# ChanghyeonKim93/nonlinear_optimizer_for_slam

Measured on AMD Instinct MI355X. Metric: ndt6_gauss_newton_residual_blocks_per_sec, higher is better.
Workload: dtype f64

## Files before the change

nonlinear_optimizer_for_slam_amd/csrc/assemble_one_launch.hpp:

```cpp
#pragma once

#include "assemble_pass.hpp"

namespace nos {

constexpr size_t kSingleBlockMaxElements = size_t(1024) * 15;

template <typename Problem, typename T, int BLOCK, bool NT>
__device__ __forceinline__ int single_block_loop(const TiledLayout& L, typename Problem::Params& P, uint32_t n_chunks,
                                                 LmDevice& s_lm, double* s_sum, double* __restrict__ cost_history,
                                                 int history_capacity) {
  constexpr int kF = Problem::kFields;
  constexpr int kOut = Problem::kOut;
  const T* __restrict__ base = static_cast<const T*>(L.base);
  int executed = 0;
  while (s_lm.st.done == 0) {
    set_pose(P, &s_lm);
    T acc[kOut];
#pragma unroll
    for (int k = 0; k < kOut; ++k) acc[k] = T(0);
    constexpr uint32_t kRound = (kF * sizeof(T) > 64) ? 2 : 4;
    for (uint32_t c = 0; c < n_chunks; c += kRound) {
      T x[kRound][kF][1];
      uint64_t i0[kRound];
#pragma unroll
      for (uint32_t u = 0; u < kRound; ++u) {
        const uint32_t cu = (c + u < n_chunks) ? c + u : c;
        i0[u] = uint64_t(cu) * BLOCK + threadIdx.x;
        const uint64_t off = (i0[u] >> L.tile_shift) * L.tile_stride + (i0[u] & L.tile_mask);
#pragma unroll
        for (int f = 0; f < kF; ++f) load_items<T, 1, NT>(base + field_offset<Problem>(L, i0[u], off, f), x[u][f]);
      }
      __builtin_amdgcn_sched_barrier(0);
#pragma unroll
      for (uint32_t u = 0; u < kRound; ++u) {
        if (c + u < n_chunks) {
          T xi[kF];
#pragma unroll
          for (int f = 0; f < kF; ++f) xi[f] = x[u][f][0];
          Problem::item(xi, P, i0[u] < L.n, acc);
        }
      }
    }
    double dacc[kOut];
#pragma unroll
    for (int k = 0; k < kOut; ++k) dacc[k] = double(acc[k]);
    block_reduce_store<kOut, BLOCK>(dacc, s_sum, false);
    __syncthreads();
    if (threadIdx.x == 0) {
      if (cost_history != nullptr && executed < history_capacity)
        __hip_atomic_store(cost_history + executed, s_sum[kOut - 1], __ATOMIC_RELAXED, __HIP_MEMORY_SCOPE_SYSTEM);
      lm_step_lane<kOut>(lds_ptr(s_sum), lds_ptr(&s_lm));
    }
    ++executed;
    __syncthreads();
  }
  return executed;
}

template <typename Problem, typename T, int BLOCK, bool NT = false>
__global__ __launch_bounds__(BLOCK) void solve_single_block_kernel(TiledLayout L, typename Problem::Params P,
                                                                  uint32_t n_chunks, LmDevice* lm,
                                                                  double* __restrict__ cost_history, int history_capacity,
                                                                  double* entry_host, unsigned long long* seq_host,
                                                                  unsigned long long seq) {
  constexpr int kOut = Problem::kOut;
  __shared__ double s_lm_raw[(sizeof(LmDevice) + 7) / 8];
  LmDevice& s_lm = *reinterpret_cast<LmDevice*>(s_lm_raw);
  __shared__ double s_sum[kLmTotDoubles(kOut)];
  if (threadIdx.x == 0) s_lm = *lm;
  __syncthreads();
  const int executed = single_block_loop<Problem, T, BLOCK, NT>(L, P, n_chunks, s_lm, s_sum, cost_history, history_capacity);
  if (threadIdx.x < kOut && entry_host != nullptr && executed > 0)
    __hip_atomic_store(entry_host + kLogOut + threadIdx.x, s_sum[threadIdx.x], __ATOMIC_RELAXED, __HIP_MEMORY_SCOPE_SYSTEM);
  if (threadIdx.x == 0) {
    const nos_host::LmState st = s_lm.st;
    lm->st = st;
    if (entry_host != nullptr) {
#pragma unroll
      for (int k = 0; k < 9; ++k)
        __hip_atomic_store(entry_host + kLogR + k, st.R[k], __ATOMIC_RELAXED, __HIP_MEMORY_SCOPE_SYSTEM);
#pragma unroll
      for (int k = 0; k < 3; ++k)
        __hip_atomic_store(entry_host + kLogT + k, st.t[k], __ATOMIC_RELAXED, __HIP_MEMORY_SCOPE_SYSTEM);
      __hip_atomic_store(entry_host + kLogLambda, st.lambda, __ATOMIC_RELAXED, __HIP_MEMORY_SCOPE_SYSTEM);
      __hip_atomic_store(entry_host + kLogPrevCost, st.previous_cost, __ATOMIC_RELAXED, __HIP_MEMORY_SCOPE_SYSTEM);
      __hip_atomic_store(entry_host + kLogCost, st.cost, __ATOMIC_RELAXED, __HIP_MEMORY_SCOPE_SYSTEM);
      __hip_atomic_store(entry_host + kLogIteration, double(st.iteration), __ATOMIC_RELAXED, __HIP_MEMORY_SCOPE_SYSTEM);
      __hip_atomic_store(entry_host + kLogDone, double(st.done), __ATOMIC_RELAXED, __HIP_MEMORY_SCOPE_SYSTEM);
      __hip_atomic_store(entry_host + kLogOk, double(st.ok), __ATOMIC_RELAXED, __HIP_MEMORY_SCOPE_SYSTEM);
      __hip_atomic_store(entry_host + kLogExecuted, double(executed), __ATOMIC_RELAXED, __HIP_MEMORY_SCOPE_SYSTEM);
    }
  }
  if (threadIdx.x < kWave) {
    asm volatile("s_waitcnt vmcnt(0)" ::: "memory");
    if (threadIdx.x == 0 && seq_host != nullptr) {
      __builtin_amdgcn_fence(__ATOMIC_RELEASE, "");
      asm volatile("s_waitcnt vmcnt(0)" ::: "memory");
      __hip_atomic_store(seq_host, seq, __ATOMIC_RELAXED, __HIP_MEMORY_SCOPE_SYSTEM);
    }
  }
}

constexpr uint32_t kClusterMaxBlocks = 256;
constexpr unsigned long long kClusterTimeoutTicks = 5000000ull;
constexpr unsigned long long kClusterMailboxTimeoutTicks = kMailboxTimeoutTicks;

struct ClusterCtl {
  unsigned int abort;
  unsigned int pad0[31];
  struct alignas(128) Arrival {
    unsigned int count;
    unsigned int pad[31];
  } arrival[8];
};

__device__ __forceinline__ double sc1_load(const double* p) {
  return __hip_atomic_load(p, __ATOMIC_RELAXED, __HIP_MEMORY_SCOPE_AGENT);
}
__device__ __forceinline__ void sc1_store(double* p, double v) {
  __hip_atomic_store(p, v, __ATOMIC_RELAXED, __HIP_MEMORY_SCOPE_AGENT);
}

__device__ __forceinline__ void state_store_sc1(LmDevice* lm, const nos_host::LmState& st) {
  double* d = reinterpret_cast<double*>(&lm->st);
  const double* s = reinterpret_cast<const double*>(&st);
  constexpr int kWords = int(sizeof(nos_host::LmState) / sizeof(double));
  static_assert(sizeof(nos_host::LmState) % sizeof(double) == 0, "LmState must be a whole number of doubles");
#pragma unroll
  for (int k = 0; k < kWords; ++k) sc1_store(d + k, s[k]);
}
__device__ __forceinline__ void state_load_sc1(const LmDevice* lm, nos_host::LmState& st) {
  const double* d = reinterpret_cast<const double*>(&lm->st);
  double* s = reinterpret_cast<double*>(&st);
  constexpr int kWords = int(sizeof(nos_host::LmState) / sizeof(double));
#pragma unroll
  for (int k = 0; k < kWords; ++k) s[k] = sc1_load(d + k);
}

template <int FIELDS, int ELEM>
struct ResidentShape;
template <>
struct ResidentShape<15, 8> { static constexpr int RI = 3, LI = 3; };
template <>
struct ResidentShape<15, 4> { static constexpr int RI = 3, LI = 4; };
template <>
struct ResidentShape<5, 8> { static constexpr int RI = 9, LI = 7; };
template <>
struct ResidentShape<5, 4> { static constexpr int RI = 10, LI = 14; };

template <typename Problem, typename T>
struct StreamRegRounds { static constexpr int kRR = 3; };
template <int LOSS>
struct StreamRegRounds<Ndt6Problem<float, LOSS>, float> { static constexpr int kRR = 0; };
constexpr int kStreamRegRoundsMax = 3;

template <typename Problem, typename T, int BLOCK, int RI, int LI, int SI = 0, bool SPF = false, bool NT = false>
__global__ __launch_bounds__(BLOCK) void solve_cluster_kernel(TiledLayout L, typename Problem::Params P,
                                                             double* __restrict__ partials, LmDevice* lm, ClusterCtl* ctl,
                                                             double* __restrict__ cost_history, int history_capacity,
                                                             double* entry_host, unsigned long long* seq_host,
                                                             unsigned long long seq, uint32_t items_per_lane,
                                                             const Mailbox* mail = nullptr, uint32_t stream_lds = 0u,
                                                             uint32_t stream_reg = 0u) {
  constexpr int kF = Problem::kFields;
  constexpr int kOut = Problem::kOut;
  constexpr int kCols = 32;
  constexpr int kSlices = BLOCK / kCols;
  const T* __restrict__ base = static_cast<const T*>(L.base);
  constexpr int kRF = kF;
  extern __shared__ __align__(16) unsigned char resident_raw[];
  T* resident = reinterpret_cast<T*>(resident_raw);
  __shared__ int s_flag;
  __shared__ int s_fast;
  __shared__ double red[kSlices][kCols];
  __shared__ double s_tot[kLmTotDoubles(kOut)];
  __shared__ double s_lmd_raw[(sizeof(LmDevice) + 7) / 8];
  LmDevice& s_lmd = *reinterpret_cast<LmDevice*>(s_lmd_raw);
  nos_host::LmState& s_state = s_lmd.st;
  [[maybe_unused]] __shared__ double s_local[kCols];
  [[maybe_unused]] __shared__ unsigned long long s_round0;
  const bool multi = mail != nullptr;

  const uint32_t J = items_per_lane & 0x7fffffffu;
  [[maybe_unused]] const bool allow_fast = (items_per_lane >> 31) == 0u;
  [[maybe_unused]] constexpr int kXccCol = 28;
  [[maybe_unused]] const unsigned int my_xcc = xcc_id();
  const uint64_t block_base = uint64_t(blockIdx.x) * BLOCK * J;
  auto fetch = [&](uint32_t j, T (&dst)[kRF]) -> bool {
    const uint64_t i = block_base + uint64_t(j) * BLOCK + threadIdx.x;
    const bool ok = i < L.n;
    const uint64_t ic = ok ? i : 0;
    const uint64_t off = (ic >> L.tile_shift) * L.tile_stride + (ic & L.tile_mask);
    T xt[kF][1];
#pragma unroll
    for (int f = 0; f < kF; ++f) load_items<T, 1, false>(base + field_offset<Problem>(L, ic, off, f), xt[f]);
#pragma unroll
    for (int f = 0; f < kF; ++f) dst[f] = ok ? xt[f][0] : T(0);
    return ok;
  };
  auto evaluate_resident = [&](const T (&xi)[kRF], bool ok, T (&acc_)[kOut]) { Problem::item(xi, P, ok, acc_); };
  T x[RI > 0 ? RI : 1][kRF];
  bool valid[RI > 0 ? RI : 1];
  static_assert(SI == 0 || (RI == 0 && LI == 0), "the streaming form keeps nothing resident");
  constexpr int kSI = SI > 0 ? SI : 1;
  [[maybe_unused]] T xs[kF][kSI];
  [[maybe_unused]] uint64_t xs_i0 = 0;
  [[maybe_unused]] constexpr int kRR = (SI > 0 && !SPF) ? StreamRegRounds<Problem, T>::kRR : 0;
  static_assert(kRR <= kStreamRegRoundsMax, "the option's range covers every instantiation");
  [[maybe_unused]] T xr[kRR > 0 ? kRR : 1][kF][kSI];
  [[maybe_unused]] const uint32_t my_rounds = blockIdx.x < J ? (J - blockIdx.x + gridDim.x - 1) / gridDim.x : 0u;
  [[maybe_unused]] const uint32_t lds_k = SI > 0 ? min(stream_lds, my_rounds > 0u ? my_rounds - 1u : 0u) : 0u;
  [[maybe_unused]] const uint32_t reg_k = kRR > 0 ? min(min(stream_reg, uint32_t(kRR)), (my_rounds > 0u ? my_rounds - 1u : 0u) - lds_k) : 0u;
  [[maybe_unused]] const uint32_t alt_k = min(lds_k, reg_k);
  [[maybe_unused]] auto chip_round = [&](uint32_t i) -> uint32_t {
    return uint32_t(uint64_t(i + 1u) * my_rounds / (lds_k + reg_k + 1u));
  };
  [[maybe_unused]] auto lds_slot_round = [&](uint32_t sl) -> uint32_t {
    return sl < lds_k ? chip_round(sl < alt_k ? 2u * sl : alt_k + sl) : ~0u;
  };
  [[maybe_unused]] const uint32_t lds_r0 = lds_slot_round(0u);
  [[maybe_unused]] const uint32_t lds_r1 = lds_slot_round(1u);
  [[maybe_unused]] const uint32_t lds_r2 = lds_slot_round(2u);
  [[maybe_unused]] uint32_t reg_r[kRR > 0 ? kRR : 1];
#pragma unroll
  for (int j = 0; j < (kRR > 0 ? kRR : 1); ++j)
    reg_r[j] = uint32_t(j) < reg_k ? chip_round(uint32_t(j) < alt_k ? 2u * uint32_t(j) + 1u : alt_k + uint32_t(j)) : ~0u;
#pragma unroll
  for (int j = 0; j < (kRR > 0 ? kRR : 1); ++j)
#pragma unroll
    for (int f = 0; f < kF; ++f)
#pragma unroll
      for (int e = 0; e < kSI; ++e) xr[j][f][e] = T(0);
  [[maybe_unused]] auto lds_round = [&](uint32_t s) -> uint32_t { return s == 0u ? lds_r0 : s == 1u ? lds_r1 : s == 2u ? lds_r2 : ~0u; };
  [[maybe_unused]] auto fetch_chunk = [&](uint32_t c, T (&dst)[kF][kSI]) -> uint64_t {
    const uint64_t i0 = uint64_t(c) * (uint64_t(BLOCK) * kSI) + uint64_t(threadIdx.x) * kSI;
    const uint64_t off = (i0 >> L.tile_shift) * L.tile_stride + (i0 & L.tile_mask);
#pragma unroll
    for (int f = 0; f < kF; ++f) load_items<T, kSI, NT>(base + field_offset<Problem>(L, i0, off, f), dst[f]);
    return i0;
  };
  if constexpr (SI > 0) {
    if (blockIdx.x < J) xs_i0 = fetch_chunk(blockIdx.x, xs);
  }
#pragma unroll
  for (int j = 0; j < RI; ++j) {
    valid[j] = false;
    if (uint32_t(j) < J) {
      valid[j] = fetch(uint32_t(j), x[j]);
    } else {
#pragma unroll
      for (int f = 0; f < kRF; ++f) x[j][f] = T(0);
    }
  }
  if constexpr (LI > 0) {
    for (uint32_t j = RI; j < J; ++j) {
      T xi[kRF];
      (void)fetch(j, xi);
#pragma unroll
      for (int f = 0; f < kRF; ++f) resident[(size_t(j - RI) * kRF + f) * BLOCK + threadIdx.x] = xi[f];
    }
  }
  NOS_PROBE(if (threadIdx.x < 4) s_step_cycles[threadIdx.x] = 0ull;)
  if (threadIdx.x == 0) {
    s_lmd.settings = lm->settings;
    s_state = lm->st;
    s_flag = s_state.done != 0 ? 1 : 0;
    s_fast = 0;
    if (__hip_atomic_load(&ctl->abort, __ATOMIC_RELAXED, __HIP_MEMORY_SCOPE_AGENT) != 0u) s_flag = 2;
    if (multi && blockIdx.x == 0) s_round0 = *mail->round;
  }
  __syncthreads();
  [[maybe_unused]] const unsigned int group = blockIdx.x & 7u;
  const unsigned int n_groups = gridDim.x < 8u ? gridDim.x : 8u;
  unsigned int it = 0;
  int executed = 0;
  NOS_PROBE(unsigned long long tq[6] = {0, 0, 0, 0, 0, 0}, tp = 0;)
#define NOS_RES_STAMP(slot_) NOS_PROBE({ const unsigned long long now_ = wall_clock64(); tq[slot_] += now_ - tp; tp = now_; })
  while (s_flag == 0) {
    NOS_PROBE(tp = wall_clock64();)
    if constexpr (kOut == 28) {
#pragma unroll
      for (int k = 0; k < 9; ++k) P.R[k] = T(uniform_load(&s_state.R[k]));
#pragma unroll
      for (int k = 0; k < 3; ++k) P.t[k] = T(uniform_load(&s_state.t[k]));
    } else {
#pragma unroll
      for (int k = 0; k < 4; ++k) P.R2[k] = T(uniform_load(&s_state.R[k]));
#pragma unroll
      for (int k = 0; k < 2; ++k) P.t2[k] = T(uniform_load(&s_state.t[k]));
    }
    T acc[kOut];
#pragma unroll
    for (int k = 0; k < kOut; ++k) acc[k] = T(0);
    if constexpr (SI > 0) {
      const uint32_t n_chunks = J;
      auto evaluate = [&](const T (&xc)[kF][SI > 0 ? SI : 1], uint64_t i0) {
#pragma unroll
        for (int it = 0; it < (SI > 0 ? SI : 1); ++it) {
          T xi[kF];
#pragma unroll
          for (int f = 0; f < kF; ++f) xi[f] = xc[f][it];
          Problem::item(xi, P, (i0 + it) < L.n, acc);
        }
      };
      if constexpr (SPF) {
        for (uint32_t c = blockIdx.x; c < n_chunks; c += gridDim.x) {
          T xb[kF][SI > 0 ? SI : 1];
          uint64_t i1 = 0;
          const uint32_t cn = c + gridDim.x;
          if (cn < n_chunks) i1 = fetch_chunk(cn, xb);
          evaluate(xs, xs_i0);
#pragma unroll
          for (int f = 0; f < kF; ++f)
#pragma unroll
            for (int it = 0; it < (SI > 0 ? SI : 1); ++it) xs[f][it] = xb[f][it];
          xs_i0 = i1;
        }
      } else {
        auto lds_at = [&](uint32_t s, int f, int e) -> T& {
          return resident[((size_t(s) * kF + f) * BLOCK + threadIdx.x) * kSI + e];
        };
        auto evaluate_lds = [&](uint32_t s, uint32_t cl) {
          const uint64_t i0 = uint64_t(cl) * (uint64_t(BLOCK) * kSI) + uint64_t(threadIdx.x) * kSI;
#pragma unroll
          for (int e = 0; e < kSI; ++e) {
            T xi[kF];
#pragma unroll
            for (int f = 0; f < kF; ++f) xi[f] = lds_at(s, f, e);
            Problem::item(xi, P, (i0 + e) < L.n, acc);
          }
        };
        const bool on_chip = it != 0u;
        uint32_t s = 0;
        uint32_t next_res = lds_round(0u);
        auto in_registers = [&](uint32_t r) -> bool {
          bool hit = false;
#pragma unroll
          for (int j = 0; j < kRR; ++j) hit = hit || r == reg_r[j];
          return hit;
        };
        uint32_t k = 0;
        if constexpr (kRR == 0) {
          while (k < my_rounds) {
            __builtin_amdgcn_sched_barrier(0);
            if (!on_chip && k == next_res) {
#pragma unroll
              for (int f = 0; f < kF; ++f)
#pragma unroll
                for (int e = 0; e < kSI; ++e) lds_at(s, f, e) = xs[f][e];
              next_res = lds_round(++s);
            }
            evaluate(xs, xs_i0);
            uint32_t kn = k + 1u;
            if (on_chip)
              for (uint32_t sn = s; kn == lds_round(sn); ++sn) ++kn;
            xs_i0 = fetch_chunk(blockIdx.x + (kn < my_rounds ? kn : 0u) * gridDim.x, xs);
            for (uint32_t kr = k + 1u; kr < kn; ++kr) {
              evaluate_lds(s, blockIdx.x + kr * gridDim.x);
              next_res = lds_round(++s);
            }
            k = kn;
          }
        } else
#pragma unroll
        for (int j = 0; j <= kRR; ++j) {
          const uint32_t rj = j < kRR ? reg_r[j < kRR ? j : 0] : ~0u;
          const uint32_t stop = min(rj, my_rounds);
          const uint32_t hi = (!on_chip && rj != ~0u) ? rj + 1u : stop;
          auto lds_rounds_below = [&](uint32_t lim) {
            while (next_res < lim) {
              evaluate_lds(s, blockIdx.x + next_res * gridDim.x);
              next_res = lds_round(++s);
            }
          };
          if (on_chip && j > 0) lds_rounds_below(min(k, stop));
          while (k < hi) {
            __builtin_amdgcn_sched_barrier(0);
            if (!on_chip) {
              if (k == next_res) {
#pragma unroll
                for (int f = 0; f < kF; ++f)
#pragma unroll
                  for (int e = 0; e < kSI; ++e) lds_at(s, f, e) = xs[f][e];
                next_res = lds_round(++s);
              }
              if constexpr (kRR > 0) {
                if (j < kRR && k == rj) {
#pragma unroll
                  for (int f = 0; f < kF; ++f)
#pragma unroll
                    for (int e = 0; e < kSI; ++e) xr[j < kRR ? j : 0][f][e] = xs[f][e];
                }
              }
            }
            evaluate(xs, xs_i0);
            uint32_t kn = k + 1u;
            if (on_chip) {
              for (uint32_t sn = s;;) {
                if (kn == lds_round(sn)) {
                  ++sn;
                  ++kn;
                } else if (in_registers(kn)) {
                  ++kn;
                } else {
                  break;
                }
              }
            }
            xs_i0 = fetch_chunk(blockIdx.x + (kn < my_rounds ? kn : 0u) * gridDim.x, xs);
            if (on_chip) lds_rounds_below(min(kn, stop));
            k = kn;
          }
          if constexpr (kRR > 0) {
            if (j < kRR && on_chip && rj != ~0u)
              evaluate(xr[j < kRR ? j : 0], uint64_t(blockIdx.x + rj * gridDim.x) * (uint64_t(BLOCK) * kSI) + uint64_t(threadIdx.x) * kSI);
          }
        }
      }
      if constexpr (SPF) {
        if (blockIdx.x < n_chunks) xs_i0 = fetch_chunk(blockIdx.x, xs);
      }
    } else
    if (sizeof(T) == 8 && J >= uint32_t(RI)) {
#pragma unroll
      for (int j = 0; j < RI; ++j) evaluate_resident(x[j], valid[j], acc);
    } else {
#pragma unroll
      for (int j = 0; j < RI; ++j)
        if (uint32_t(j) < J) evaluate_resident(x[j], valid[j], acc);
    }
    if constexpr (LI > 0) {
      for (uint32_t j = RI; j < J; ++j) {
        T xi[kRF];
#pragma unroll
        for (int f = 0; f < kRF; ++f) xi[f] = resident[(size_t(j - RI) * kRF + f) * BLOCK + threadIdx.x];
        evaluate_resident(xi, (block_base + uint64_t(j) * BLOCK + threadIdx.x) < L.n, acc);
      }
    }
    double dacc[kOut];
#pragma unroll
    for (int k = 0; k < kOut; ++k) dacc[k] = double(acc[k]);
    NOS_RES_STAMP(0)
    {
      TaggedUnit* const block_units = reinterpret_cast<TaggedUnit*>(partials);
      TaggedUnit* const group_units = block_units + size_t(kClusterMaxBlocks) * 32;
      const unsigned long long tag = (seq << 24) | ((unsigned long long)it + 1ull);
      const double mine = block_reduce_value<kOut, BLOCK>(dacc);
      const bool probe = it == 0u && allow_fast;
      if (threadIdx.x < kOut) {
        if (s_fast != 0)
          tagged_store_plain(block_units + size_t(blockIdx.x) * 32 + threadIdx.x, mine, tag);
        else
          tagged_store(block_units + size_t(blockIdx.x) * 32 + threadIdx.x, mine, tag);
      } else if (probe && threadIdx.x == kXccCol) {
        tagged_store(block_units + size_t(blockIdx.x) * 32 + kXccCol, double(my_xcc), tag);
      }
      NOS_RES_STAMP(1)
      const unsigned long long deadline = wall_clock64() + (multi ? kClusterMailboxTimeoutTicks : kClusterTimeoutTicks);
      auto await = [&](const TaggedUnit* u, double* value) -> bool {
        unsigned int polls = 0;
        for (;;) {
          const TaggedUnit got = tagged_load(u);
          if (got.seq == tag) {
            *value = got.value;
            return true;
          }
          if ((++polls & 63u) == 0u &&
              (__hip_atomic_load(&ctl->abort, __ATOMIC_RELAXED, __HIP_MEMORY_SCOPE_AGENT) != 0u || wall_clock64() > deadline)) {
            __hip_atomic_store(&ctl->abort, 1u, __ATOMIC_RELAXED, __HIP_MEMORY_SCOPE_AGENT);
            s_flag = 2;
            return false;
          }
        }
      };
      const int col = threadIdx.x % kCols;
      const int slice = threadIdx.x / kCols;
      if (blockIdx.x < n_groups) {
        const unsigned int g_size = (gridDim.x - blockIdx.x + 7u) >> 3;
        double gsum = 0.0;
        for (unsigned int m0 = 0; m0 < g_size; m0 += kSlices) {
          const unsigned int m = m0 + slice;
          double v = 0.0;
          if (m < g_size && (col < kOut || (probe && col == kXccCol))) {
            (void)await(block_units + size_t(blockIdx.x + 8u * m) * 32 + col, &v);
            if (col == kXccCol) v = v == double(my_xcc) ? 0.0 : 1.0;
          }
          red[slice][col] = v;
          __syncthreads();
          if (threadIdx.x < kOut || (probe && threadIdx.x == kXccCol)) {
#pragma unroll
            for (int sl = 0; sl < kSlices; ++sl) gsum += red[sl][threadIdx.x];
          }
          __syncthreads();
        }
        if ((threadIdx.x < kOut || (probe && threadIdx.x == kXccCol)) && s_flag != 2)
          tagged_store(group_units + (size_t(it & 1u) * 8 + blockIdx.x) * 32 + threadIdx.x, gsum, tag);
      }
      if (!multi || blockIdx.x == 0) {
        double v = 0.0;
        if (slice < int(n_groups) && (col < kOut || (probe && col == kXccCol)) && s_flag != 2)
          (void)await(group_units + (size_t(it & 1u) * 8 + slice) * 32 + col, &v);
        if (slice < 8) red[slice][col] = v;
      }
      __syncthreads();
      if (multi) {
        TaggedUnit* const global_units = group_units + size_t(2) * 8 * 32;
        if (blockIdx.x == 0) {
          if (threadIdx.x < kCols && s_flag != 2) {
            double tot = 0.0;
            if (threadIdx.x < kOut || (probe && threadIdx.x == kXccCol))
              for (unsigned int g = 0; g < n_groups; ++g) tot += red[g][threadIdx.x];
            s_local[threadIdx.x] = tot;
          }
          __syncthreads();
          if (threadIdx.x < kWave) {
            const Mailbox mb = *mail;
            const unsigned long long round = s_round0 + (unsigned long long)it + 1ull;
            const unsigned int xtag = (unsigned int)(round % 0xFFFFFFFFull) + 1u;
            const size_t parity = size_t(round & 1ull);
            const size_t units_base = size_t(mb.n_ranks) * 2 * kMailSlotDoubles;
            const int lane = int(threadIdx.x);
            const bool giving_up = s_flag == 2;
            unsigned long long* const own = reinterpret_cast<unsigned long long*>(mb.peers[mb.rank] + units_base);
            if (giving_up) {
              if (lane < mb.n_ranks)
                __hip_atomic_store(reinterpret_cast<unsigned long long*>(mb.peers[lane] + units_base) +
                                       (size_t(mb.rank) * 2 + parity) * kMailSlotDoubles + 63,
                                   (unsigned long long)xtag << 32, __ATOMIC_RELAXED, __HIP_MEMORY_SCOPE_SYSTEM);
            } else {
              unsigned long long gran = 0ull;
              if (lane < 2 * kOut) {
                const unsigned long long bits = (unsigned long long)__double_as_longlong(s_local[lane >> 1]);
                gran = ((unsigned long long)xtag << 32) | ((lane & 1) ? (bits >> 32) : (bits & 0xFFFFFFFFull));
                for (int p = 0; p < mb.n_ranks; ++p)
                  __hip_atomic_store(reinterpret_cast<unsigned long long*>(mb.peers[p] + units_base) +
                                         (size_t(mb.rank) * 2 + parity) * kMailSlotDoubles + lane,
                                     gran, __ATOMIC_RELAXED, __HIP_MEMORY_SCOPE_SYSTEM);
              }
              double sum = 0.0;
              bool lost = false;
              const unsigned long long give_up_at = wall_clock64() + kClusterMailboxTimeoutTicks;
              for (int r = 0; r < mb.n_ranks && !lost; ++r) {
                const unsigned long long* slot_r = own + (size_t(r) * 2 + parity) * kMailSlotDoubles;
                unsigned long long got = 0ull;
                unsigned int polls = 0;
                for (;;) {
                  if (lane < 2 * kOut) got = __hip_atomic_load(slot_r + lane, __ATOMIC_RELAXED, __HIP_MEMORY_SCOPE_SYSTEM);
                  const bool here = lane >= 2 * kOut || (unsigned int)(got >> 32) == xtag;
                  if (__ballot(!here) == 0ull) break;
                  if ((++polls & 15u) == 0u) {
                    const unsigned long long peer_gave_up =
                        __hip_atomic_load(slot_r + 63, __ATOMIC_RELAXED, __HIP_MEMORY_SCOPE_SYSTEM);
                    if ((unsigned int)(peer_gave_up >> 32) == xtag || wall_clock64() > give_up_at ||
                        __hip_atomic_load(&ctl->abort, __ATOMIC_RELAXED, __HIP_MEMORY_SCOPE_AGENT) != 0u) {
                      lost = true;
                      break;
                    }
                  }
                  __builtin_amdgcn_s_sleep(1);
                }
                const unsigned int half = (unsigned int)(got & 0xFFFFFFFFull);
                const unsigned int other = (unsigned int)__shfl_xor(int(half), 1, kWave);
                const double value = __longlong_as_double((long long)(((unsigned long long)((lane & 1) ? half : other) << 32) |
                                                                      (unsigned long long)((lane & 1) ? other : half)));
                sum += value;
              }
              if (lost) {
                if (lane == 0) {
                  __hip_atomic_store(&ctl->abort, 1u, __ATOMIC_RELAXED, __HIP_MEMORY_SCOPE_AGENT);
                  s_flag = 2;
                }
                if (lane < mb.n_ranks)
                  __hip_atomic_store(reinterpret_cast<unsigned long long*>(mb.peers[lane] + units_base) +
                                         (size_t(mb.rank) * 2 + parity) * kMailSlotDoubles + 63,
                                     (unsigned long long)xtag << 32, __ATOMIC_RELAXED, __HIP_MEMORY_SCOPE_SYSTEM);
              } else if (lane < 2 * kOut && (lane & 1) == 0) {
                s_local[lane >> 1] = sum;
              }
            }
          }
          __syncthreads();
          if (s_flag != 2) {
            if (threadIdx.x < kOut || (probe && threadIdx.x == kXccCol))
              tagged_store(global_units + size_t(it & 1u) * 32 + threadIdx.x, s_local[threadIdx.x], tag);
          }
        }
        {
          double v = 0.0;
          if (threadIdx.x < kCols && (col < kOut || (probe && col == kXccCol)) && s_flag != 2)
            (void)await(global_units + size_t(it & 1u) * 32 + col, &v);
          if (threadIdx.x < kCols) red[0][col] = v;
        }
        __syncthreads();
      }
      NOS_RES_STAMP(2)
      if (s_flag == 2) break;
      if (multi) {
        if (threadIdx.x < kOut)
          s_tot[threadIdx.x] = red[0][threadIdx.x];
        else if (probe && threadIdx.x == kXccCol)
          s_fast = red[0][kXccCol] == 0.0 ? 1 : 0;
      } else
      if (threadIdx.x < kOut) {
        double tot = 0.0;
        for (unsigned int g = 0; g < n_groups; ++g) tot += red[g][threadIdx.x];
        s_tot[threadIdx.x] = tot;
      } else if (probe && threadIdx.x == kXccCol) {
        double strangers = 0.0;
        for (unsigned int g = 0; g < n_groups; ++g) strangers += red[g][kXccCol];
        s_fast = strangers == 0.0 ? 1 : 0;
      }
      __syncthreads();
    }
    {
      NOS_RES_STAMP(3)
      if (threadIdx.x == 0) {
        if (blockIdx.x == 0 && cost_history != nullptr && executed < history_capacity)
          __hip_atomic_store(cost_history + executed, s_tot[kOut - 1], __ATOMIC_RELAXED, __HIP_MEMORY_SCOPE_SYSTEM);
        lm_step_lane<kOut>(lds_ptr(s_tot), lds_ptr(&s_lmd));
        s_flag = s_state.done != 0 ? 1 : 0;
      }
    }
    ++executed;
    ++it;
    __syncthreads();
    NOS_RES_STAMP(4)
  }
  NOS_PROBE(
  if (blockIdx.x == 0 && threadIdx.x == 0 && entry_host != nullptr) {
    for (int k = 0; k < 5; ++k)
      __hip_atomic_store(entry_host + 50 + k, double(tq[k]) / double(executed > 0 ? executed : 1), __ATOMIC_RELAXED,
                         __HIP_MEMORY_SCOPE_SYSTEM);
    for (int k = 0; k < 3; ++k)
      __hip_atomic_store(entry_host + 56 + k, double(s_step_cycles[k]) / double(executed > 0 ? executed : 1), __ATOMIC_RELAXED,
                         __HIP_MEMORY_SCOPE_SYSTEM);
  }
  )
  if (s_flag == 1 && blockIdx.x == 0) {
    if (threadIdx.x < kOut && entry_host != nullptr && executed > 0)
      __hip_atomic_store(entry_host + kLogOut + threadIdx.x, s_tot[threadIdx.x], __ATOMIC_RELAXED, __HIP_MEMORY_SCOPE_SYSTEM);
    if (threadIdx.x == 0) {
      const nos_host::LmState st = s_state;
      lm->st = st;
      if (multi) *mail->round = s_round0 + (unsigned long long)executed;
      if (entry_host != nullptr) {
#pragma unroll
        for (int k = 0; k < 9; ++k)
          __hip_atomic_store(entry_host + kLogR + k, st.R[k], __ATOMIC_RELAXED, __HIP_MEMORY_SCOPE_SYSTEM);
#pragma unroll
        for (int k = 0; k < 3; ++k)
          __hip_atomic_store(entry_host + kLogT + k, st.t[k], __ATOMIC_RELAXED, __HIP_MEMORY_SCOPE_SYSTEM);
        __hip_atomic_store(entry_host + kLogLambda, st.lambda, __ATOMIC_RELAXED, __HIP_MEMORY_SCOPE_SYSTEM);
        __hip_atomic_store(entry_host + kLogPrevCost, st.previous_cost, __ATOMIC_RELAXED, __HIP_MEMORY_SCOPE_SYSTEM);
        __hip_atomic_store(entry_host + kLogCost, st.cost, __ATOMIC_RELAXED, __HIP_MEMORY_SCOPE_SYSTEM);
        __hip_atomic_store(entry_host + kLogIteration, double(st.iteration), __ATOMIC_RELAXED, __HIP_MEMORY_SCOPE_SYSTEM);
        __hip_atomic_store(entry_host + kLogDone, double(st.done), __ATOMIC_RELAXED, __HIP_MEMORY_SCOPE_SYSTEM);
        __hip_atomic_store(entry_host + kLogOk, double(st.ok), __ATOMIC_RELAXED, __HIP_MEMORY_SCOPE_SYSTEM);
        __hip_atomic_store(entry_host + kLogExecuted, double(executed), __ATOMIC_RELAXED, __HIP_MEMORY_SCOPE_SYSTEM);
      }
    }
    if (threadIdx.x < kWave) {
      asm volatile("s_waitcnt vmcnt(0)" ::: "memory");
      if (threadIdx.x == 0 && seq_host != nullptr) {
        __builtin_amdgcn_fence(__ATOMIC_RELEASE, "");
        asm volatile("s_waitcnt vmcnt(0)" ::: "memory");
        __hip_atomic_store(seq_host, seq, __ATOMIC_RELAXED, __HIP_MEMORY_SCOPE_SYSTEM);
      }
    }
  }
}

}
```

Before: 76.60 billion.

## Use single merged streaming loop for register/LDS-resident rounds in NDT kernels

Adds a single-loop path for NDT3 and NDT6 problems. On the first iteration it stashes chunks into LDS or register slots. On later iterations it walks all rounds in order, interleaving reads from LDS and registers with prefetched global chunks, instead of running a separate loop segment per register round. It also turns on one register-resident round for float NDT6. The aim is to cut loop-segment overhead and keep the global prefetch overlapped, at the cost of more register pressure and dynamic selection among the register slots.

Result: no change. 76.93 billion (median of 4 runs) (+0.4%).

```diff
diff --git a/nonlinear_optimizer_for_slam_amd/csrc/assemble_one_launch.hpp b/nonlinear_optimizer_for_slam_amd/csrc/assemble_one_launch.hpp
--- a/nonlinear_optimizer_for_slam_amd/csrc/assemble_one_launch.hpp
+++ b/nonlinear_optimizer_for_slam_amd/csrc/assemble_one_launch.hpp
@@ -150,9 +150,13 @@
 struct ResidentShape<5, 4> { static constexpr int RI = 10, LI = 14; };
 
 template <typename Problem, typename T>
-struct StreamRegRounds { static constexpr int kRR = 3; };
+struct StreamRegRounds { static constexpr int kRR = 3; static constexpr bool kSingleLoop = false; };
+template <typename T, int LOSS>
+struct StreamRegRounds<Ndt3Problem<T, LOSS>, T> { static constexpr int kRR = 3; static constexpr bool kSingleLoop = true; };
 template <int LOSS>
-struct StreamRegRounds<Ndt6Problem<float, LOSS>, float> { static constexpr int kRR = 0; };
+struct StreamRegRounds<Ndt6Problem<double, LOSS>, double> { static constexpr int kRR = 3; static constexpr bool kSingleLoop = true; };
+template <int LOSS>
+struct StreamRegRounds<Ndt6Problem<float, LOSS>, float> { static constexpr int kRR = 1; static constexpr bool kSingleLoop = true; };
 constexpr int kStreamRegRoundsMax = 3;
 
 template <typename Problem, typename T, int BLOCK, int RI, int LI, int SI = 0, bool SPF = false, bool NT = false>
@@ -362,6 +366,82 @@
             }
             k = kn;
           }
+        } else if constexpr (StreamRegRounds<Problem, T>::kSingleLoop) {
+          if (!on_chip) {
+            while (k < my_rounds) {
+              __builtin_amdgcn_sched_barrier(0);
+              if (k == next_res) {
+#pragma unroll
+                for (int f = 0; f < kF; ++f)
+#pragma unroll
+                  for (int e = 0; e < kSI; ++e) lds_at(s, f, e) = xs[f][e];
+                next_res = lds_round(++s);
+              }
+#pragma unroll
+              for (int j = 0; j < kRR; ++j) {
+                if (k == reg_r[j]) {
+#pragma unroll
+                  for (int f = 0; f < kF; ++f)
+#pragma unroll
+                    for (int e = 0; e < kSI; ++e) xr[j][f][e] = xs[f][e];
+                }
+              }
+              evaluate(xs, xs_i0);
+              ++k;
+              xs_i0 = fetch_chunk(blockIdx.x + (k < my_rounds ? k : 0u) * gridDim.x, xs);
+            }
+          }
+          uint32_t jr = 0;
+          auto reg_round = [&](uint32_t j) -> uint32_t {
+            uint32_t r = ~0u;
+#pragma unroll
+            for (int jj = 0; jj < kRR; ++jj) r = j == uint32_t(jj) ? reg_r[jj] : r;
+            return r;
+          };
+          uint32_t next_reg = reg_round(0u);
+          while (k < my_rounds) {
+            __builtin_amdgcn_sched_barrier(0);
+            evaluate(xs, xs_i0);
+            uint32_t kn = k + 1u;
+            {
+              uint32_t sa = s, ja = jr, ra = next_res, ga = next_reg;
+              while (kn == ra || kn == ga) {
+                if (kn == ra)
+                  ra = lds_round(++sa);
+                else
+                  ga = reg_round(++ja);
+                ++kn;
+              }
+            }
+            xs_i0 = fetch_chunk(blockIdx.x + (kn < my_rounds ? kn : 0u) * gridDim.x, xs);
+            for (uint32_t kr = k + 1u; kr < kn; ++kr) {
+              T xc[kF][kSI];
+              if (kr == next_res) {
+#pragma unroll
+                for (int f = 0; f < kF; ++f)
+#pragma unroll
+                  for (int e = 0; e < kSI; ++e) xc[f][e] = lds_at(s, f, e);
+                next_res = lds_round(++s);
+              } else {
+#pragma unroll
+                for (int f = 0; f < kF; ++f)
+#pragma unroll
+                  for (int e = 0; e < kSI; ++e) xc[f][e] = xr[0][f][e];
+#pragma unroll
+                for (int j = 1; j < kRR; ++j) {
+                  if (jr == uint32_t(j)) {
+#pragma unroll
+                    for (int f = 0; f < kF; ++f)
+#pragma unroll
+                      for (int e = 0; e < kSI; ++e) xc[f][e] = xr[j][f][e];
+                  }
+                }
+                next_reg = reg_round(++jr);
+              }
+              evaluate(xc, uint64_t(blockIdx.x + kr * gridDim.x) * (uint64_t(BLOCK) * kSI) + uint64_t(threadIdx.x) * kSI);
+            }
+            k = kn;
+          }
         } else
 #pragma unroll
         for (int j = 0; j <= kRR; ++j) {
```
